# Themaister/Granite

Hardware: AMD Instinct MI355X
Metric: Mpixels/s for clustered-light+post chain @4K; achieved HBM GB/s vs roofline (higher is better)
Workload: dtype f32

## Files before the change

granite_amd/capi.py:

```python
from __future__ import annotations

import ctypes as C
import os
from typing import Optional

import numpy as np

_HERE = os.path.dirname(os.path.abspath(__file__))
LIB_PATH = os.path.join(_HERE, os.environ.get("GRANITE_LIB_DIR", "lib"), "libgranite_hip.so")

FORMAT_R8_UNORM = 9
FORMAT_R8G8_UNORM = 16
FORMAT_R8G8B8A8_UNORM = 37
FORMAT_R8G8B8A8_SRGB = 43
FORMAT_B8G8R8A8_UNORM = 44
FORMAT_B8G8R8A8_SRGB = 50
FORMAT_A2B10G10R10_UNORM_PACK32 = 64
FORMAT_R16_UNORM = 70
FORMAT_R16_SFLOAT = 76
FORMAT_R16G16_UNORM = 77
FORMAT_R16G16_SFLOAT = 83
FORMAT_R16G16B16A16_SFLOAT = 97
FORMAT_R32_SFLOAT = 100
FORMAT_R32G32_SFLOAT = 103
# ... 7 lines not shown
FORMAT_BC2_UNORM_BLOCK = 135
FORMAT_BC2_SRGB_BLOCK = 136
FORMAT_BC3_UNORM_BLOCK = 137
FORMAT_BC3_SRGB_BLOCK = 138
FORMAT_BC4_UNORM_BLOCK = 139
FORMAT_BC5_UNORM_BLOCK = 141
FORMAT_BC6H_UFLOAT_BLOCK = 143
FORMAT_BC6H_SFLOAT_BLOCK = 144
FORMAT_BC7_UNORM_BLOCK = 145
FORMAT_BC7_SRGB_BLOCK = 146
BLOCK_FORMATS = (131, 132, 133, 134, 135, 136, 137, 138, 139, 141, 143, 144, 145, 146)
FORMAT_ASTC_4x4_UNORM_BLOCK = 157
FORMAT_ASTC_4x4_SRGB_BLOCK = 158
FORMAT_ASTC_5x4_UNORM_BLOCK = 159
FORMAT_ASTC_5x4_SRGB_BLOCK = 160
FORMAT_ASTC_5x5_UNORM_BLOCK = 161
FORMAT_ASTC_5x5_SRGB_BLOCK = 162
FORMAT_ASTC_6x5_UNORM_BLOCK = 163
FORMAT_ASTC_6x5_SRGB_BLOCK = 164
FORMAT_ASTC_6x6_UNORM_BLOCK = 165
FORMAT_ASTC_6x6_SRGB_BLOCK = 166
FORMAT_ASTC_8x5_UNORM_BLOCK = 167
FORMAT_ASTC_8x5_SRGB_BLOCK = 168
FORMAT_ASTC_8x6_UNORM_BLOCK = 169
FORMAT_ASTC_8x6_SRGB_BLOCK = 170
FORMAT_ASTC_8x8_UNORM_BLOCK = 171
FORMAT_ASTC_8x8_SRGB_BLOCK = 172
FORMAT_ASTC_10x5_UNORM_BLOCK = 173
FORMAT_ASTC_10x5_SRGB_BLOCK = 174
FORMAT_ASTC_10x6_UNORM_BLOCK = 175
FORMAT_ASTC_10x6_SRGB_BLOCK = 176
FORMAT_ASTC_10x8_UNORM_BLOCK = 177
FORMAT_ASTC_10x8_SRGB_BLOCK = 178
FORMAT_ASTC_10x10_UNORM_BLOCK = 179
FORMAT_ASTC_10x10_SRGB_BLOCK = 180
FORMAT_ASTC_12x10_UNORM_BLOCK = 181
FORMAT_ASTC_12x10_SRGB_BLOCK = 182
FORMAT_ASTC_12x12_UNORM_BLOCK = 183
FORMAT_ASTC_12x12_SRGB_BLOCK = 184
ASTC_FOOTPRINTS = ((4, 4), (5, 4), (5, 5), (6, 5), (6, 6), (8, 5), (8, 6), (8, 8), (10, 5), (10, 6), (10, 8), (10, 10), (12, 10), (12, 12))
ASTC_FORMATS = {157 + i: ASTC_FOOTPRINTS[i // 2] for i in range(28)}

FORMAT_BPP = {
    FORMAT_R8_UNORM: 1,
    FORMAT_R8G8_UNORM: 2,
    FORMAT_R8G8B8A8_UNORM: 4,
    FORMAT_R8G8B8A8_SRGB: 4,
    FORMAT_B8G8R8A8_UNORM: 4,
    FORMAT_B8G8R8A8_SRGB: 4,
    FORMAT_R16_UNORM: 2,
    FORMAT_R16G16_UNORM: 4,
    FORMAT_A2B10G10R10_UNORM_PACK32: 4,
    FORMAT_R16_SFLOAT: 2,
    FORMAT_R16G16_SFLOAT: 4,
    FORMAT_R16G16B16A16_SFLOAT: 8,
    FORMAT_R32_SFLOAT: 4,
    FORMAT_R32G32_SFLOAT: 8,
    FORMAT_B10G11R11_UFLOAT_PACK32: 4,
    FORMAT_D16_UNORM: 2,
    FORMAT_D32_SFLOAT: 4,
}

COLOR_SPACE_SRGB_NONLINEAR = 0
COLOR_SPACE_EXTENDED_SRGB_LINEAR = 1000104002
COLOR_SPACE_HDR10_ST2084 = 1000104008
VIDEO_CONTROL_SKIP_RESCALE_BIT = 1
VIDEO_CONTROL_DOWNSCALING_BIT = 2
VIDEO_CONTROL_SAMPLED_DOWNSCALING_BIT = 4
VIDEO_CONTROL_CLAMP_COORD_BIT = 8
VIDEO_CONTROL_CHROMA_SUBSAMPLE_BIT = 16
VIDEO_CONTROL_PRIMARY_CONVERSION_BIT = 32
VIDEO_CONTROL_DITHER_BIT = 64
VIDEO_TRANSFER_IDENTITY = 0
VIDEO_TRANSFER_SRGB = 1
VIDEO_TRANSFER_PQ = 2
VIDEO_MATRIX_UNSPECIFIED, VIDEO_MATRIX_BT601_525, VIDEO_MATRIX_BT601_625, VIDEO_MATRIX_BT709, VIDEO_MATRIX_BT2020, VIDEO_MATRIX_SMPTE240M = range(6)
VIDEO_CHROMA_CENTER, VIDEO_CHROMA_LEFT, VIDEO_CHROMA_TOPLEFT, VIDEO_CHROMA_TOP, VIDEO_CHROMA_BOTTOMLEFT, VIDEO_CHROMA_BOTTOM = range(6)

LIGHTING_DIRECTIONAL_BIT = 1
LIGHTING_CLUSTERED_BIT = 2
LIGHTING_AMBIENT_FALLBACK_BIT = 4
LIGHTING_AMBIENT_OCCLUSION_BIT = 8
LIGHTING_SHARE_REGISTERS_BIT = 16

MAX_LIGHTS_BINDLESS = 4096
CULL_SETUP_BYTES_PER_LIGHT = 512
TRANSFORMED_SPOT_BYTES_PER_LIGHT = 96
TRANSFORMS_OFFSET_LIGHTS = 0
TRANSFORMS_OFFSET_SHADOW = 196608
TRANSFORMS_OFFSET_MODEL = 458752
TRANSFORMS_OFFSET_TYPE_MASK = 655360
TRANSFORMS_OFFSET_DECALS = 655872
TRANSFORMS_SIZE = 852480


class Cube(C.Structure):
    _fields_ = [("ptr", C.c_void_p), ("size", C.c_uint32), ("levels", C.c_uint32)]


class Image(C.Structure):
    _fields_ = [("ptr", C.c_void_p), ("width", C.c_uint32), ("height", C.c_uint32), ("pitch_bytes", C.c_uint32),
                ("format", C.c_uint32)]


FFT_FORWARD_C2C, FFT_INVERSE_C2C, FFT_R2C, FFT_C2R = 0, 1, 2, 3
FFT_FP32, FFT_FP16 = 0, 1
FFT_RESOURCE_TEXTURE, FFT_RESOURCE_BUFFER = 0, 1
FFT_PASS_C2C, FFT_PASS_R2C_RESOLVE, FFT_PASS_C2R_RESOLVE = 0, 1, 2
FFT_BUFFER_SRC, FFT_BUFFER_DST, FFT_BUFFER_SCRATCH_A, FFT_BUFFER_SCRATCH_B = 0, 1, 2, 3


class FftOptions(C.Structure):
    _fields_ = [("nx", C.c_uint32), ("ny", C.c_uint32), ("nz", C.c_uint32), ("dimensions", C.c_uint32), ("mode", C.c_uint32),
                ("data_type", C.c_uint32), ("input_resource", C.c_uint32), ("output_resource", C.c_uint32)]


class FftResource(C.Structure):
    _fields_ = [("type", C.c_uint32), ("ptr", C.c_void_p), ("size_bytes", C.c_uint64), ("row_stride", C.c_uint32), ("layer_stride", C.c_uint32),
                ("image", Image), ("output_offset", C.c_int32 * 2)]


class FftPass(C.Structure):
    _fields_ = [("kind", C.c_uint32), ("dimension", C.c_uint32), ("points", C.c_uint32), ("p", C.c_uint32), ("columns", C.c_uint32),
                ("workgroup_size", C.c_uint32), ("grid_size", C.c_uint32), ("lds_bytes", C.c_uint32), ("reads", C.c_uint32), ("writes", C.c_uint32)]


class PushVideo(C.Structure):
    _fields_ = [("resolution", C.c_int32 * 2), ("scaling_to_input", C.c_float * 2), ("inv_input_resolution", C.c_float * 2),
                ("dither_strength", C.c_float)]


assert C.sizeof(PushVideo) == 28


class VideoPlan(C.Structure):
    _fields_ = [("flags", C.c_uint32), ("eotf", C.c_uint32), ("oetf", C.c_uint32), ("num_planes", C.c_uint32), ("push", PushVideo),
                ("gamma_space_transform", C.c_float * 12), ("primary_transform", C.c_float * 9)]


class PushYuvToRgb(C.Structure):
    _fields_ = [("yuv_to_rgb", C.c_float * 16), ("primary_conversion", C.c_float * 16), ("resolution", C.c_uint32 * 2),
                ("inv_resolution", C.c_float * 2), ("chroma_siting", C.c_float * 2), ("chroma_clamp", C.c_float * 2),
                ("unorm_rescale", C.c_float)]


assert C.sizeof(PushYuvToRgb) == 164


class VideoYuvInfo(C.Structure):
    _fields_ = [("bit_depth", C.c_uint32), ("msb_aligned", C.c_uint32), ("full_range", C.c_uint32), ("matrix", C.c_uint32),
                ("chroma_location", C.c_uint32), ("pq", C.c_uint32), ("nv21", C.c_uint32)]


class VideoYuvPlan(C.Structure):
    _fields_ = [("push", PushYuvToRgb), ("spec_pq", C.c_uint32), ("spec_num_planes", C.c_uint32), ("spec_nv21", C.c_uint32),
                ("matrix", C.c_uint32)]


OCEAN_VARIANT_HEIGHT, OCEAN_VARIANT_GRADIENT_NORMAL, OCEAN_VARIANT_GRADIENT_DISPLACEMENT = 0, 1, 2
OCEAN_NUM_FREQ_BANDS = 8


class PushOceanGenerate(C.Structure):
    _fields_ = [("mod_factor", C.c_float * 2), ("N", C.c_uint32 * 2), ("freq_to_band_mod", C.c_float), ("time", C.c_float), ("period", C.c_float)]


# ... 1054 lines not shown
```

granite_amd/csrc/lighting.hip:

```cpp
#include <cstdlib>
#include <cstring>
#include "ctx.hpp"
#include "device_common.hpp"

namespace
{
constexpr int LIGHT_TILE = 8;
#ifndef LV_WAVES
#define LV_WAVES 4
#endif
constexpr int LIGHT_WAVES = LV_WAVES;
constexpr int LIGHT_SLOT_BYTES = 64;

constexpr float PI_SIC = 3.1415628f;
constexpr float CULL_RADIUS_SCALE = 1.001f;
constexpr float CULL_SLACK = 1e-3f;

#ifdef LV_STAMP
#define LV_STAMP_PARAM , uint32_t (&stamp_marks__)[4]
#define LV_STAMP_ARG , stamp_scope__.marks
#define LV_STAMP_MARK(k) stamp_marks__[k] = uint32_t(__builtin_amdgcn_s_memtime())
#define LV_STAMP_LAP_BEGIN() uint32_t stamp_lap__ = uint32_t(__builtin_amdgcn_s_memtime())
#define LV_STAMP_LAP(k)                                                          \
	do                                                                           \
// ... 75 lines not shown
__device__ __forceinline__ void brdf_accumulate(const Surface &s, float NdL, float hh, float scale, float3_ colour, float3_ &acc)
{
	const float NoL = med3(NdL, 0.001f, 1.0f);
	const float inv_h = rsq(hh);
	const float omh = sat(fmaf(-0.5f * hh, inv_h, 1.001f)) - 0.001f;
	const float NoH = sat((s.NdV + NdL) * inv_h);

	const float omh2 = omh * omh;
	const float f = omh2 * omh2 * omh;

	const float d = fmaf(NoH * NoH, s.m2m1, 1.0f);
	const float g = fmaf(NoL, s.gA, s.gB);
	const float GD = rcp(d * d * g);

	const float w = NoL * scale;
	const float cw = fmaf(-f, w, w);
	const float fw = f * GD * w;
	acc.x = fmaf(colour.x, fmaf(fmaf(GD, s.F0.x, s.D1.x), cw, fw), acc.x);
	acc.y = fmaf(colour.y, fmaf(fmaf(GD, s.F0.y, s.D1.y), cw, fw), acc.y);
	acc.z = fmaf(colour.z, fmaf(fmaf(GD, s.F0.z, s.D1.z), cw, fw), acc.z);
}

__device__ __forceinline__ bool index_in_range(uint32_t index, uint32_t range_x, uint32_t range_y)
{
	return index >= range_x && index <= range_y;
}

template <bool IS_MAX>
__device__ __forceinline__ uint32_t minmax_step(uint32_t v, uint32_t moved)
{
	return IS_MAX ? max(v, moved) : min(v, moved);
}
#define GR_DPP_STEP(IS_MAX, v, ctrl) v = minmax_step<IS_MAX>(v, uint32_t(__builtin_amdgcn_mov_dpp(int(v), ctrl, 0xf, 0xf, true)))
#define GR_DPP_BCAST(IS_MAX, v, ctrl, rows) \
	v = minmax_step<IS_MAX>(v, uint32_t(__builtin_amdgcn_update_dpp(IS_MAX ? 0 : -1, int(v), ctrl, rows, 0xf, false)))
template <bool IS_MAX>
__device__ __forceinline__ uint32_t wave_minmax_u32(uint32_t v)
{
	GR_DPP_STEP(IS_MAX, v, 0xB1);
	GR_DPP_STEP(IS_MAX, v, 0x4E);
	GR_DPP_STEP(IS_MAX, v, 0x141);
	GR_DPP_STEP(IS_MAX, v, 0x140);
	GR_DPP_BCAST(IS_MAX, v, 0x142, 0xa);
	GR_DPP_BCAST(IS_MAX, v, 0x143, 0xc);
	return uint32_t(__builtin_amdgcn_readlane(int(v), 63));
}
__device__ __forceinline__ void wave_min_and_max_u32(uint32_t &lo, uint32_t &hi)
{
	GR_DPP_STEP(false, lo, 0xB1);
	GR_DPP_STEP(true, hi, 0xB1);
	GR_DPP_STEP(false, lo, 0x4E);
	GR_DPP_STEP(true, hi, 0x4E);
	GR_DPP_STEP(false, lo, 0x141);
	GR_DPP_STEP(true, hi, 0x141);
	GR_DPP_STEP(false, lo, 0x140);
	GR_DPP_STEP(true, hi, 0x140);
	GR_DPP_BCAST(false, lo, 0x142, 0xa);
	GR_DPP_BCAST(true, hi, 0x142, 0xa);
	GR_DPP_BCAST(false, lo, 0x143, 0xc);
	GR_DPP_BCAST(true, hi, 0x143, 0xc);
	lo = uint32_t(__builtin_amdgcn_readlane(int(lo), 63));
	hi = uint32_t(__builtin_amdgcn_readlane(int(hi), 63));
}
#undef GR_DPP_STEP
#undef GR_DPP_BCAST

__device__ __forceinline__ uint32_t wave_inclusive_add_u32(uint32_t v)
{
	v += uint32_t(__builtin_amdgcn_update_dpp(0, int(v), 0x111, 0xf, 0xf, true));
	v += uint32_t(__builtin_amdgcn_update_dpp(0, int(v), 0x112, 0xf, 0xf, true));
	v += uint32_t(__builtin_amdgcn_update_dpp(0, int(v), 0x114, 0xf, 0xf, true));
	v += uint32_t(__builtin_amdgcn_update_dpp(0, int(v), 0x118, 0xf, 0xf, true));
	v += uint32_t(__builtin_amdgcn_update_dpp(0, int(v), 0x142, 0xa, 0xf, false));
	v += uint32_t(__builtin_amdgcn_update_dpp(0, int(v), 0x143, 0xc, 0xf, false));
	return v;
}
__device__ __forceinline__ uint32_t bits_from(uint32_t index, uint32_t word_first)
{
	return index <= word_first ? 0xffffffffu : (index - word_first >= 32u ? 0u : 0xffffffffu << (index - word_first));
}

extern __shared__ __attribute__((aligned(16))) uint8_t lv_dynamic_lds[];

template <int PX, bool CONE>
__device__ __forceinline__ void shade_positional(const Surface (&s)[PX], const f32x4 *slot, float3_ (&result)[PX])
{
	const f32x4 q0 = slot[0], q1 = slot[1];
	float3_ Lf[PX];
	float d2[PX];
	bool near_any = false;
#pragma unroll
	for (int p = 0; p < PX; p++)
	{
		Lf[p] = f3(q0.x, q0.y, q0.z) - s[p].pos;
		d2[p] = fmaf(Lf[p].z, Lf[p].z, fmaf(Lf[p].y, Lf[p].y, fmaf(Lf[p].x, Lf[p].x, 1e-30f)));
		near_any = near_any || d2[p] < q0.w;
	}
	if (!__any(near_any))
		return;

	float inv_d[PX], len[PX], inv_d2[PX], atten[PX];
#pragma unroll
	for (int p = 0; p < PX; p++)
	{
		inv_d[p] = rsq(d2[p]);
		len[p] = d2[p] * inv_d[p];
		const float dist = CONE ? fmaxf(0.1f, len[p]) : len[p];
		inv_d2[p] = inv_d[p] * inv_d[p];
		const float t = sat(fmaf(dist, q1.w, -9.0f));
		atten[p] = fmaf(t * t, fmaf(2.0f, t, -3.0f), 1.0f);
	}
	if (CONE)
	{
		const f32x4 q2 = slot[2], q3 = slot[3];
		bool lit_any = false;
#pragma unroll
		for (int p = 0; p < PX; p++)
		{
			const float cone_angle = -dot(Lf[p], f3(q2.x, q2.y, q2.z)) * inv_d[p];
			const float cone = sat(fmaf(cone_angle, q3.x, q3.y));
			atten[p] *= cone * cone;
			lit_any = lit_any || atten[p] > 0.0f;
		}
		if (!__any(lit_any))
			return;
	}
#pragma unroll
	for (int p = 0; p < PX; p++)
	{
		const float a2 = atten[p] * fminf(inv_d2[p], 1.0f / (0.1f * 0.1f));
		const float NdL = dot(s[p].N, Lf[p]) * inv_d[p];
		const float3_ Hs = f3(fmaf(s[p].V.x, len[p], Lf[p].x), fmaf(s[p].V.y, len[p], Lf[p].y), fmaf(s[p].V.z, len[p], Lf[p].z));
		const float hh = fmaf(Hs.z, Hs.z, fmaf(Hs.y, Hs.y, fmaf(Hs.x, Hs.x, 1e-30f))) * inv_d2[p];
		brdf_accumulate(s[p], NdL, hh, a2, f3(q1.x, q1.y, q1.z), result[p]);
	}
}


template <int PX, bool B10>
struct RawTile
{
	float depth[PX];
	uint32_t alb[PX], nrm[PX];
	uint32_t mr;
	uint32_t em[B10 ? PX : 2 * PX];
};

template <int PX, bool B10>
__device__ __forceinline__ void load_raw(const KernelArgs &a, int x0, int y, RawTile<PX, B10> &r)
{
	const uint32_t uy = uint32_t(min(y, a.hdr.h - 1)), ux = uint32_t(min(x0, a.hdr.w - PX));
	if constexpr (PX == 2)
	{
		const float2 d = *reinterpret_cast<const float2 *>(a.depth.ptr + (uy * a.depth.pitch + ux * 4u));
		const uint2 al = *reinterpret_cast<const uint2 *>(a.albedo.ptr + (uy * a.albedo.pitch + ux * 4u));
		const uint2 nr = *reinterpret_cast<const uint2 *>(a.normal.ptr + (uy * a.normal.pitch + ux * 4u));
		r.mr = *reinterpret_cast<const uint32_t *>(a.pbr.ptr + (uy * a.pbr.pitch + ux * 2u));
		if constexpr (B10)
		{
			const uint2 packed = *reinterpret_cast<const uint2 *>(a.emissive.ptr + (uy * a.emissive.pitch + ux * 4u));
			r.em[0] = packed.x, r.em[1] = packed.y;
		}
		else
		{
			const uint4 em = *reinterpret_cast<const uint4 *>(a.emissive.ptr + (uy * a.emissive.pitch + ux * 8u));
			r.em[0] = em.x, r.em[1] = em.y, r.em[2] = em.z, r.em[3] = em.w;
		}
		r.depth[0] = d.x, r.depth[PX - 1] = d.y;
		r.alb[0] = al.x, r.alb[PX - 1] = al.y;
		r.nrm[0] = nr.x, r.nrm[PX - 1] = nr.y;
	}
	else
	{
		r.depth[0] = *reinterpret_cast<const float *>(a.depth.ptr + (uy * a.depth.pitch + ux * 4u));
		r.alb[0] = *reinterpret_cast<const uint32_t *>(a.albedo.ptr + (uy * a.albedo.pitch + ux * 4u));
		r.nrm[0] = *reinterpret_cast<const uint32_t *>(a.normal.ptr + (uy * a.normal.pitch + ux * 4u));
		r.mr = *reinterpret_cast<const uint16_t *>(a.pbr.ptr + (uy * a.pbr.pitch + ux * 2u));
		if constexpr (B10)
			r.em[0] = *reinterpret_cast<const uint32_t *>(a.emissive.ptr + (uy * a.emissive.pitch + ux * 4u));
		else
		{
			const uint2 em = *reinterpret_cast<const uint2 *>(a.emissive.ptr + (uy * a.emissive.pitch + ux * 8u));
			r.em[0] = em.x, r.em[1] = em.y;
		}
	}
}


template <int PX, bool B10>
__device__ __forceinline__ void unpack_raw(const RawTile<PX, B10> &raw, float (&depth)[PX], uint32_t (&alb)[PX], uint32_t (&nrm)[PX], uint32_t (&mr)[PX],
                                           f16x4 (&dst)[PX])
{
#pragma unroll
	for (int p = 0; p < PX; p++)
	{
		depth[p] = raw.depth[p];
		alb[p] = raw.alb[p];
		nrm[p] = raw.nrm[p];
		mr[p] = PX == 2 ? (p == 0 ? raw.mr & 0xffffu : raw.mr >> 16) : raw.mr;
		if constexpr (B10)
		{
			uint32_t rg, ba;
			expand_b10g11r11(raw.em[p], rg, ba);
			dst[p] = __builtin_bit_cast(f16x4, make_uint2(rg, ba));
		}
		else
			dst[p] = __builtin_bit_cast(f16x4, make_uint2(raw.em[2 * p], raw.em[2 * p + 1]));
	}
}

template <bool B10, int CHANNEL>
__device__ __forceinline__ float blend_round(float v)
{
// ... 52 lines not shown
		const float3_ L = f3(a.dir_direction[0], a.dir_direction[1], a.dir_direction[2]);
		const float3_ Hv = s.V + L;
		float3_ lit = f3(0.0f, 0.0f, 0.0f);
		brdf_accumulate(s, dot(s.N, L), fmaxf(dot(Hv, Hv), 1e-30f), 1.0f, f3(a.dir_color[0], a.dir_color[1], a.dir_color[2]), lit);
		float ambient = (a.flags & GR_LIGHTING_AMBIENT_FALLBACK_BIT) ? 0.05f : 0.0f;
		if (AO)
			ambient *= sample_linear_r8(a.ao, (float(x) + 0.5f) * a.inv_resolution[0], (float(y) + 0.5f) * a.inv_resolution[1]);
		lit = f3(fmaf(base.x, ambient, lit.x), fmaf(base.y, ambient, lit.y), fmaf(base.z, ambient, lit.z));
		accum = f3(blend_round<B10, 0>(accum.x + lit.x), blend_round<B10, 1>(accum.y + lit.y), blend_round<B10, 2>(accum.z + lit.z));
	}
}

struct Cells { int cx0, cx1, cy0, cy1; };

__device__ __forceinline__ int cluster_cell(int p, float inv_res, float scale, int res)
{
	return clamp0_i32(int(__fmul_rn(__fmul_rn(float(p) + 0.5f, inv_res), scale)), res - 1);
}

template <int PX>
__device__ __forceinline__ Cells tile_cells(const KernelArgs &a, const int x0, const int y, const int lane)
{
	const int my_cx = cluster_cell(min(x0 + (lane >> 5) * (PX - 1), a.hdr.w - 1), a.inv_resolution[0], a.cl_xy_scale[0], a.cl_res_x);
	const int my_cy = cluster_cell(min(y, a.hdr.h - 1), a.inv_resolution[1], a.cl_xy_scale[1], a.cl_res_y);
	const int cx0 = __builtin_amdgcn_readlane(my_cx, 0), cx1 = __builtin_amdgcn_readlane(my_cx, 63);
	const int cy0 = __builtin_amdgcn_readlane(my_cy, 0), cy1 = __builtin_amdgcn_readlane(my_cy, 63);
	return {cx0, cx1, cy0, cy1};
}

template <int PX>
__device__ __forceinline__ void bounding_sphere(const bool (&member)[PX], const Surface (&s)[PX], float3_ &centre_out, float &radius_out)
{
	bool any_member = false;
#pragma unroll
	for (int p = 0; p < PX; p++)
		any_member = any_member || member[p];
	const int first = __builtin_ctzll(__ballot(any_member));
	const float3_ mine = PX == 2 && !member[0] ? s[PX - 1].pos : s[0].pos;
	centre_out = f3(__builtin_bit_cast(float, __builtin_amdgcn_readlane(__builtin_bit_cast(int, mine.x), first)),
	                __builtin_bit_cast(float, __builtin_amdgcn_readlane(__builtin_bit_cast(int, mine.y), first)),
	                __builtin_bit_cast(float, __builtin_amdgcn_readlane(__builtin_bit_cast(int, mine.z), first)));
	float off2 = 0.0f;
#pragma unroll
	for (int p = 0; p < PX; p++)
	{
		const float3_ off = s[p].pos - centre_out;
		const float mine2 = member[p] ? dot(off, off) : 0.0f;
		off2 = p == 0 ? mine2 : fmaxf(off2, mine2);
	}
	radius_out = __builtin_amdgcn_sqrtf(__builtin_bit_cast(float, wave_minmax_u32<true>(__builtin_bit_cast(uint32_t, off2)))) * 1.0001f + CULL_SLACK;
}

__device__ __forceinline__ void or_cell_words(const KernelArgs &a, const Cells &cells, const int my_word, uint32_t &word)
{
	for (int cy = cells.cy0; cy <= cells.cy1; cy++)
	{
#pragma clang loop vectorize(disable) unroll(disable)
		for (int cx = cells.cx0; cx <= cells.cx1; cx++)
			word |= a.bitmask[(cy * a.cl_res_x + cx) * a.cl_num_lights_32 + my_word];
	}
}

__device__ __forceinline__ int gather_wide(const KernelArgs &a, const Cells &cells, const uint32_t win_lo, const uint32_t win_hi, const uint32_t gap_lo,
                                           const uint32_t gap_hi, const int span_word, const int word_last, const int lane, uint16_t *const list)
{
	const int my_word = span_word + lane;
	const uint32_t word_first = uint32_t(my_word) << 5u;
	uint32_t word = 0u;
	if (lane < a.list_words && my_word <= word_last)
	{
		or_cell_words(a, cells, my_word, word);
		word &= bits_from(win_lo, word_first) & ~bits_from(win_hi + 1u, word_first) & ~(bits_from(gap_lo + 1u, word_first) & ~bits_from(gap_hi, word_first));
	}
	const uint32_t count = uint32_t(__builtin_popcount(word));
	const uint32_t upto = wave_inclusive_add_u32(count);
	const int list_count = __builtin_amdgcn_readlane(int(upto), 63);
	uint16_t *entry = list + (upto - count);
	for (; word != 0u; word &= word - 1u)
		*entry++ = uint16_t(word_first + uint32_t(__builtin_ctz(word)));
	__builtin_amdgcn_wave_barrier();
	return list_count;
}

__device__ __forceinline__ void cull_and_stage(const KernelArgs &a, const uint32_t light_index, const float3_ &centre, const float tile_radius, const int lane,
                                               f32x4 *const slots, bool &keep, bool &second)
{
	const f32x4 *rec = reinterpret_cast<const f32x4 *>(a.lights + light_index);
	const f32x4 c = rec[0], pq = rec[1], d = rec[2];
	const float radius = CULL_RADIUS_SCALE * rcp(d.w);
	const float3_ to_light = f3(pq.x, pq.y, pq.z) - centre;
	const float reach = radius + tile_radius;
	const float dist2 = dot(to_light, to_light);
	keep = dist2 <= reach * reach;
	const bool is_spot = ((a.type_mask[light_index >> 5] >> (light_index & 31u)) & 1u) == 0u;
	const float sb_lane = c.w;
	const uint32_t sb_bits = __builtin_bit_cast(uint32_t, sb_lane);
	const float spot_scale = float(__builtin_bit_cast(_Float16, uint16_t(sb_bits & 0xffffu)));
	const float spot_bias = float(__builtin_bit_cast(_Float16, uint16_t(sb_bits >> 16)));
	if (is_spot && keep && spot_scale > 0.0f)
	{
		const float cos_t = -spot_bias * rcp(spot_scale);
		if (cos_t > 0.0f && cos_t < 1.0f)
		{
			const float sin_t = __builtin_amdgcn_sqrtf(fmaf(-cos_t, cos_t, 1.0f));
			const float along = -dot(to_light, f3(d.x, d.y, d.z));
			const float off_axis = __builtin_amdgcn_sqrtf(fmaxf(fmaf(-along, along, dist2), 0.0f));
			const float e = fmaf(off_axis, cos_t, -along * sin_t);
			keep = e <= tile_radius * 1.001f + CULL_SLACK;
		}
	}
	second = is_spot || d.w > 8.0f;
	if (keep)
	{
		f32x4 *dst_slot = slots + lane * (LIGHT_SLOT_BYTES / 16);
		dst_slot[0] = f32x4{pq.x, pq.y, pq.z, radius * radius};
		dst_slot[1] = f32x4{c.x, c.y, c.z, 10.0f * d.w};
		if (second)
		{
			dst_slot[2] = is_spot ? f32x4{d.x, d.y, d.z, 0.0f} : f32x4{0.0f, 0.0f, 0.0f, 0.0f};
			dst_slot[3] = is_spot ? f32x4{spot_scale, spot_bias, 0.0f, 0.0f} : f32x4{0.0f, 1.0f, 0.0f, 0.0f};
		}
	}
}

template <int PX, bool CONE>
__device__ __forceinline__ void walk_next(uint64_t &todo, const Surface (&s)[PX], const f32x4 *const slots, float3_ (&result)[PX])
{
	const int bit = __builtin_ctzll(todo);
	asm("s_bitset0_b64 %0, %1" : "+s"(todo) : "s"(bit));
	shade_positional<PX, CONE>(s, slots + bit * (LIGHT_SLOT_BYTES / 16), result);
}

template <int PX, bool AO, bool B10>
__device__ __forceinline__ void shade_tile(const KernelArgs &a, const int tile_x0, const int tile_y0, const int wave, const int lane, const RawTile<PX, B10> &raw,
                                           f32x4 *const slots, const float *s_srgb LV_STAMP_PARAM)
{
	const int x0 = tile_x0 + (lane & (LIGHT_TILE - 1)) * PX;
	const int y = tile_y0 + (lane >> 3);
	const int W = a.hdr.w;
	const bool row_inside = y >= a.row_first && y < a.row_end;

	bool inside[PX], active[PX];
#pragma unroll
	for (int p = 0; p < PX; p++)
		inside[p] = row_inside && x0 + p < W;
	f16x4 dst[PX];
	float depth[PX];
	uint32_t alb[PX], nrm[PX], mr[PX];
	unpack_raw<PX, B10>(raw, depth, alb, nrm, mr, dst);
	float clip_base[4];
	{
		const float ndc_x = fmaf(2.0f * (float(x0) + 0.5f), a.inv_resolution[0], -1.0f);
		const float ndc_y = fmaf(2.0f * (float(y) + 0.5f), a.inv_resolution[1], -1.0f);
#pragma unroll
		for (int i = 0; i < 4; i++)
			clip_base[i] = fmaf(a.inv_vp[4 + i], ndc_y, fmaf(a.inv_vp[i], ndc_x, a.inv_vp[12 + i]));
	}

	Surface s[PX];
	float3_ accum[PX];
	bool any_active = false;
#pragma unroll
	for (int p = 0; p < PX; p++)
	{
		active[p] = inside[p] && depth[p] != 0.0f;
		any_active = any_active || active[p];
		float3_ base, N;
		float metallic, mat_roughness;
		decode_gbuffer(alb[p], nrm[p], mr[p], s_srgb, base, N, metallic, mat_roughness);
		float clip[4];
#pragma unroll
		for (int i = 0; i < 4; i++)
			clip[i] = fmaf(depth[p], a.inv_vp[8 + i], p == 0 ? clip_base[i] : clip_base[i] + float(p) * a.clip_dx[i]);
		make_surface(a, clip, active[p], N, base, metallic, mat_roughness, s[p]);
		accum[p] = f3(float(dst[p].x), float(dst[p].y), float(dst[p].z));
		directional_quad<AO, B10>(a, s[p], base, x0 + p, y, accum[p]);
	}

	LV_STAMP_MARK(0);
	f16x4 out_h[PX];
	float3_ out_f[PX];
	if ((a.flags & GR_LIGHTING_CLUSTERED_BIT) && a.cl_num_lights > 0)
	{
		float3_ result[PX];
		uint32_t lane_lo = 0xffffffffu, lane_hi = 0u;
		uint2 px_range[PX];
#pragma unroll
		for (int p = 0; p < PX; p++)
		{
			result[p] = f3(0.0f, 0.0f, 0.0f);
			const float zf = fmaf(s[p].pos.z, a.cl_z_row[2], fmaf(s[p].pos.y, a.cl_z_row[1], fmaf(s[p].pos.x, a.cl_z_row[0], a.cl_z_row[3])));
			const uint32_t z_index = uint32_t(clamp0_i32(int(zf), a.cl_z_max_index));
			if (active[p])
			{
				const uint2 z_range = *reinterpret_cast<const uint2 *>(reinterpret_cast<const uint8_t *>(a.range) + (z_index << 3u));
				px_range[p] = z_range;
				lane_lo = min(lane_lo, z_range.x);
				lane_hi = max(lane_hi, z_range.y);
			}
		}
		wave_min_and_max_u32(lane_lo, lane_hi);
		const uint32_t win_lo = lane_lo, win_hi = min(lane_hi, uint32_t(a.cl_num_lights - 1));
		const bool wide = a.list_words != 0 && win_lo <= win_hi && (win_hi >> 6u) - (win_lo >> 6u) >= 2u;
		uint32_t gap_lo = 0u, gap_hi = 0xffffffffu;
		bool in_low[PX], in_high[PX];
#pragma unroll
		for (int p = 0; p < PX; p++)
			in_low[p] = in_high[p] = false;
		if (wide)
		{
			uint32_t first_end = 0xffffffffu;
#pragma unroll
			for (int p = 0; p < PX; p++)
				first_end = min(first_end, active[p] && px_range[p].x <= px_range[p].y ? px_range[p].y : 0xffffffffu);
			first_end = wave_minmax_u32<false>(first_end);
#pragma unroll
			for (int p = 0; p < PX; p++)
			{
				const bool some = active[p] && px_range[p].x <= px_range[p].y, low = px_range[p].x <= first_end;
				in_low[p] = some && low, in_high[p] = some && !low;
				gap_lo = max(gap_lo, some && low ? px_range[p].y : 0u);
				gap_hi = min(gap_hi, some && !low ? px_range[p].x : 0xffffffffu);
			}
			wave_min_and_max_u32(gap_hi, gap_lo);
		}
		if (win_lo <= win_hi)
		{
			const Cells cells = tile_cells<PX>(a, x0, y, lane);
			float3_ centre;
			float tile_radius;
			bounding_sphere<PX>(active, s, centre, tile_radius);

			LV_STAMP_MARK(1);
			LV_STAMP_LAP_BEGIN();
			const int chunk_lo = int(win_lo >> 6u), chunk_hi = int(win_hi >> 6u);
			auto turn = [&](const uint32_t light_index, const bool candidate, const float3_ &centre, const float tile_radius) __attribute__((always_inline)) {
				bool keep = false, second = false;
				if (candidate)
					cull_and_stage(a, light_index, centre, tile_radius, lane, slots, keep, second);
				const uint64_t kept = __ballot(keep);
				const uint64_t seconds = __ballot(keep && second);
				__builtin_amdgcn_wave_barrier();
				LV_STAMP_LAP(2);

				for (uint64_t todo = kept & ~seconds; todo != 0ull;)
					walk_next<PX, false>(todo, s, slots, result);
				for (uint64_t todo = seconds; todo != 0ull;)
					walk_next<PX, true>(todo, s, slots, result);
				LV_STAMP_LAP(3);
				__builtin_amdgcn_wave_barrier();
			};
			if (!wide)
			{
				for (int chunk = chunk_lo; chunk <= chunk_hi; chunk++)
				{
					const uint32_t light_index = uint32_t(chunk) * 64u + uint32_t(lane);
					const int my_word = chunk * 2 + (lane >> 5);
					bool candidate = false;
					if (index_in_range(light_index, win_lo, win_hi))
					{
						uint32_t word = 0u;
						or_cell_words(a, cells, my_word, word);
						candidate = ((word >> (uint32_t(lane) & 31u)) & 1u) != 0u;
					}
					turn(light_index, candidate, centre, tile_radius);
				}
			}
			else
			{
				const bool two_groups = gap_hi != 0xffffffffu && gap_hi > gap_lo + 1u;
				float3_ centre_low = centre, centre_high = centre;
				float radius_low = tile_radius, radius_high = tile_radius;
				if (two_groups)
				{
					bounding_sphere<PX>(in_low, s, centre_low, radius_low);
					bounding_sphere<PX>(in_high, s, centre_high, radius_high);
				}
				uint16_t *const list = reinterpret_cast<uint16_t *>(lv_dynamic_lds) + wave * (a.list_words * 32);
				const int word_last = int(win_hi >> 5u);
				for (int span_word = int(win_lo >> 5u); span_word <= word_last; span_word += a.list_words)
				{
					const int list_count = gather_wide(a, cells, win_lo, win_hi, gap_lo, gap_hi, span_word, word_last, lane, list);
					for (int next = 0; next < list_count; next += 64)
					{
						const bool candidate = next + lane < list_count;
						const uint32_t light_index = candidate ? uint32_t(list[next + lane]) : 0u;
						const bool upper = light_index >= gap_hi;
						turn(light_index, candidate,
						     f3(upper ? centre_high.x : centre_low.x, upper ? centre_high.y : centre_low.y, upper ? centre_high.z : centre_low.z),
						     upper ? radius_high : radius_low);
					}
					__builtin_amdgcn_wave_barrier();
				}
			}
		}
#pragma unroll
		for (int p = 0; p < PX; p++)
		{
			out_f[p] = f3(accum[p].x + result[p].x, accum[p].y + result[p].y, accum[p].z + result[p].z);
			out_h[p].x = _Float16(out_f[p].x);
			out_h[p].y = _Float16(out_f[p].y);
			out_h[p].z = _Float16(out_f[p].z);
		}
	}
	else
	{
#pragma unroll
		for (int p = 0; p < PX; p++)
		{
			out_f[p] = accum[p];
			out_h[p].x = _Float16(accum[p].x);
			out_h[p].y = _Float16(accum[p].y);
			out_h[p].z = _Float16(accum[p].z);
		}
	}

	if (!inside[0])
		return;
	f16x4 o[PX];
#pragma unroll
	for (int p = 0; p < PX; p++)
	{
		o[p] = dst[p];
		if (active[p])
		{
			o[p].x = out_h[p].x;
			o[p].y = out_h[p].y;
			o[p].z = out_h[p].z;
		}
	}
	if (a.fog_falloff > 0.0f)
	{
#pragma unroll
		for (int p = 0; p < PX; p++)
			if (active[p])
			{
				const float3_ eye = s[p].pos - f3(a.camera_pos[0], a.camera_pos[1], a.camera_pos[2]);
				const float f = __builtin_amdgcn_exp2f(-dot(eye, eye) * a.fog_falloff), omf = 1.0f - f;
				const float3_ lit = B10 ? f3(round_to_ufloat<6>(out_f[p].x), round_to_ufloat<6>(out_f[p].y), round_to_ufloat<5>(out_f[p].z))
				                        : f3(float(o[p].x), float(o[p].y), float(o[p].z));
				out_f[p] = f3(fmaf(lit.x, f, a.fog_color[0] * omf), fmaf(lit.y, f, a.fog_color[1] * omf), fmaf(lit.z, f, a.fog_color[2] * omf));
				o[p].x = _Float16(out_f[p].x);
				o[p].y = _Float16(out_f[p].y);
				o[p].z = _Float16(out_f[p].z);
				o[p].w = _Float16(fmaf(float(dst[p].w), f, f * omf));
			}
	}
	if constexpr (B10)
	{
		if (any_active || a.emissive.ptr != a.hdr.ptr)
		{
			uint32_t words[PX];
#pragma unroll
			for (int p = 0; p < PX; p++)
				words[p] = active[p] ? pack_b10g11r11(out_f[p].x, out_f[p].y, out_f[p].z) : pack_b10g11r11(float(dst[p].x), float(dst[p].y), float(dst[p].z));
			uint8_t *out = a.hdr.ptr + (uint32_t(y) * a.hdr.pitch + uint32_t(x0) * 4u);
			if constexpr (PX == 2)
				*reinterpret_cast<uint2 *>(out) = make_uint2(words[0], words[PX - 1]);
			else
				*reinterpret_cast<uint32_t *>(out) = words[0];
		}
		return;
	}
	if (any_active || a.emissive.ptr != a.hdr.ptr)
	{
		uint8_t *out = a.hdr.ptr + (uint32_t(y) * a.hdr.pitch + uint32_t(x0) * 8u);
		if constexpr (PX == 2)
		{
			const uint2 lo = __builtin_bit_cast(uint2, o[0]), hi = __builtin_bit_cast(uint2, o[PX - 1]);
			*reinterpret_cast<uint4 *>(out) = make_uint4(lo.x, lo.y, hi.x, hi.y);
		}
		else
			*reinterpret_cast<f16x4 *>(out) = o[0];
// ... 22 lines not shown
		asm volatile("s_getreg_b32 %0, hwreg(HW_REG_HW_ID)" : "=s"(hw));
		if (rec && (threadIdx.x & 63u) == 0u)
		{
			rec[0] = make_uint4(uint32_t(t0), uint32_t(t1), uint32_t(c1 - c0), (xcc << 28) | (hw & 0x0fffffffu));
			rec[1] = make_uint4(marks[0] ? marks[0] - uint32_t(c0) : 0u, marks[1] ? marks[1] - uint32_t(c0) : 0u, marks[2], marks[3]);
		}
	}
};
#define LV_STAMP_SCOPE(tile) StampScope stamp_scope__{uint32_t(tile)}
#else
#define LV_STAMP_SCOPE(tile)
#endif

#ifdef LV_WAVES_PER_EU
#define LV_OCCUPANCY_ATTR __attribute__((amdgpu_waves_per_eu(LV_WAVES_PER_EU, LV_WAVES_PER_EU)))
#else
#define LV_OCCUPANCY_ATTR
#endif
template <int PX, bool AO, bool B10 = false>
__global__ __launch_bounds__(64 * LIGHT_WAVES) LV_OCCUPANCY_ATTR void k_lighting(KernelArgs a)
{
	__shared__ __attribute__((aligned(16))) f32x4 s_lights[LIGHT_WAVES][64 * (LIGHT_SLOT_BYTES / 16)];
	__shared__ float s_srgb[256];
	constexpr int TILE_W = LIGHT_TILE * PX;
#pragma unroll
	for (int i = 0; i < 256; i += 64 * LIGHT_WAVES)
		s_srgb[i + threadIdx.x] = a.srgb_lut[i + threadIdx.x];
	const int wave = __builtin_amdgcn_readfirstlane(int(threadIdx.x >> 6));
	const int lane = threadIdx.x & 63;
	const int tile_x0 = (int(blockIdx.x) * LIGHT_WAVES + wave) * TILE_W, tile_y0 = (a.block_row0 + int(blockIdx.y)) * LIGHT_TILE;
	LV_STAMP_SCOPE((int(blockIdx.y) * int(gridDim.x) + int(blockIdx.x)) * LIGHT_WAVES + wave);
	RawTile<PX, B10> raw;
	load_raw<PX, B10>(a, tile_x0 + (lane & (LIGHT_TILE - 1)) * PX, tile_y0 + (lane >> 3), raw);
	__syncthreads();
	shade_tile<PX, AO, B10>(a, tile_x0, tile_y0, wave, lane, raw, s_lights[threadIdx.x >> 6], s_srgb LV_STAMP_ARG);
}

KernelArgs fill_kernel_args(const gr_lighting_args *args, const gr_ctx *ctx, const bool clustered)
{
	KernelArgs k{};
	k.albedo = to_dev(&args->albedo);
	k.normal = to_dev(&args->normal);
	k.pbr = to_dev(&args->pbr);
	k.depth = to_dev(&args->depth);
	k.emissive = to_dev(&args->emissive);
	if (args->flags & GR_LIGHTING_AMBIENT_OCCLUSION_BIT)
		k.ao = to_dev(&args->ambient_occlusion);
	k.hdr = to_dev_rw(&args->hdr);
	for (int i = 0; i < 16; i++)
		k.inv_vp[i] = args->inv_view_projection[i];
	for (int i = 0; i < 4; i++)
		k.clip_dx[i] = k.inv_vp[i] * (2.0f * args->clustering.inv_resolution[0]);
	for (int i = 0; i < 3; i++)
	{
		k.camera_pos[i] = args->clustering.camera_pos[i];
		k.dir_color[i] = args->directional.color[i];
		k.dir_direction[i] = args->directional.direction[i];
	}
	k.inv_resolution[0] = args->clustering.inv_resolution[0];
	k.inv_resolution[1] = args->clustering.inv_resolution[1];
	k.cl_xy_scale[0] = args->cluster.xy_scale[0];
	k.cl_xy_scale[1] = args->cluster.xy_scale[1];
	k.cl_res_x = args->cluster.resolution_xy[0];
	k.cl_res_y = args->cluster.resolution_xy[1];
	k.cl_num_lights = clustered ? args->cluster.num_lights : 0;
	k.cl_num_lights_32 = args->cluster.num_lights_32;
	k.cl_z_max_index = args->cluster.z_max_index;
	{
		const float *front = args->cluster.camera_front, *camera = args->cluster.camera_base;
		const double z_scale = args->cluster.z_scale;
		for (int i = 0; i < 3; i++)
			k.cl_z_row[i] = float(double(front[i]) * z_scale);
		k.cl_z_row[3] = float(-(double(camera[0]) * front[0] + double(camera[1]) * front[1] + double(camera[2]) * front[2]) * z_scale);
	}
	if (clustered)
	{
		const uint8_t *t = static_cast<const uint8_t *>(args->transforms);
		k.lights = reinterpret_cast<const gr_light_info *>(t + GR_TRANSFORMS_OFFSET_LIGHTS);
		k.type_mask = reinterpret_cast<const uint32_t *>(t + GR_TRANSFORMS_OFFSET_TYPE_MASK);
		k.bitmask = args->bitmask;
		k.range = reinterpret_cast<const uint2 *>(args->range);
	}
	k.srgb_lut = ctx->srgb_decode_lut;
	k.flags = args->flags & (GR_LIGHTING_DIRECTIONAL_BIT | GR_LIGHTING_CLUSTERED_BIT | GR_LIGHTING_AMBIENT_FALLBACK_BIT | GR_LIGHTING_AMBIENT_OCCLUSION_BIT);
	for (int i = 0; i < 3; i++)
		k.fog_color[i] = args->fog_color[i];
	k.fog_falloff = args->fog_falloff > 0.0f ? args->fog_falloff : 0.0f;
	return k;
}

struct LdsPolicy
{
	size_t pad_lds;
	int list_words;
};
LdsPolicy lds_policy(const int px, const uint32_t flags)
{
	static const int max_wgs_env = []() {
		const char *env = gr_measurement_switch("GR_LIGHTING_WGS_PER_CU");
		const int v = env ? atoi(env) : 0;
		return v >= 1 && v <= 8 ? v : 0;
	}();
	const int max_wgs = max_wgs_env ? max_wgs_env : (px == 2 ? ((flags & GR_LIGHTING_SHARE_REGISTERS_BIT) ? 4 : 5) : 7);
	const size_t static_lds = sizeof(f32x4) * LIGHT_WAVES * 64 * (LIGHT_SLOT_BYTES / 16) + 256 * sizeof(float);
	const size_t per_wg = ((160u - 8u) * 1024u / unsigned(max_wgs * 4 / LIGHT_WAVES)) & ~size_t(1023);
	LdsPolicy lds{max_wgs >= 8 || per_wg <= static_lds ? 0 : per_wg - static_lds, 0};
	static const int pad_kib = []() { const char *env = gr_measurement_switch("GR_LIGHTING_PAD_KIB"); return env ? atoi(env) : -1; }();
	if (pad_kib >= 0)
		lds.pad_lds = size_t(pad_kib) * 1024u;
	const size_t words = lds.pad_lds / (size_t(LIGHT_WAVES) * 32u * sizeof(uint16_t));
	static const bool narrow_only = []() { const char *env = gr_measurement_switch("GR_LIGHTING_NARROW_ONLY"); return env && atoi(env) != 0; }();
	if (words >= 8 && !narrow_only)
		lds.list_words = int(words < 64 ? words : 64);
	return lds;
}

}

extern "C" {

int gr_lighting(gr_ctx *ctx, gr_stream stream, const gr_lighting_args *args)
{
	if (!ctx)
		return GR_ERR_INVALID_ARGUMENT;
	GR_CHECK_ARG(ctx, args != nullptr);
	GR_CHECK_IMAGE(ctx, &args->hdr, GR_HDR_FORMATS);
	const uint32_t W = args->hdr.width, H = args->hdr.height;
	const bool b10 = args->hdr.format == GR_FORMAT_B10G11R11_UFLOAT_PACK32;
	const uint32_t hdr_bpp = gr_format_texel_bytes(args->hdr.format);
	GR_CHECK_IMAGE(ctx, &args->emissive, args->hdr.format, W, H);
	GR_CHECK_IMAGE(ctx, &args->albedo, GR_FORMAT_R8G8B8A8_SRGB, W, H);
	GR_CHECK_IMAGE(ctx, &args->normal, GR_FORMAT_A2B10G10R10_UNORM_PACK32, W, H);
	GR_CHECK_IMAGE(ctx, &args->pbr, GR_FORMAT_R8G8_UNORM, W, H);
	GR_CHECK_IMAGE(ctx, &args->depth, GR_FORMAT_D32_SFLOAT, W, H);
	const bool clustered = (args->flags & GR_LIGHTING_CLUSTERED_BIT) != 0 && args->cluster.num_lights > 0;
	if (clustered)
	{
		GR_CHECK_ARG(ctx, args->transforms && args->bitmask && args->range);
		GR_CHECK_ARG(ctx, args->cluster.num_lights <= GR_MAX_LIGHTS_BINDLESS);
		GR_CHECK_ARG(ctx, args->cluster.resolution_xy[0] > 0 && args->cluster.resolution_xy[1] > 0);
	}

	const bool ao = (args->flags & GR_LIGHTING_AMBIENT_OCCLUSION_BIT) != 0;
	if (ao)
	{
		GR_CHECK_ARG(ctx, (args->flags & GR_LIGHTING_AMBIENT_FALLBACK_BIT) != 0);
		GR_CHECK_IMAGE(ctx, &args->ambient_occlusion, GR_FORMAT_R8_UNORM);
	}
	const RowSpan span = resolve_rows(args->rows.count ? &args->rows : nullptr, H);
	if (span.count() == 0)
		return GR_OK;
	GR_CHECK_ARG(ctx, uint64_t(args->hdr.pitch_bytes) * H <= 0xffffffffull && uint64_t(args->emissive.pitch_bytes) * H <= 0xffffffffull);

	KernelArgs k = fill_kernel_args(args, ctx, clustered);
	k.row_first = int(span.first);
	k.row_end = int(span.end);
	k.block_row0 = int(span.first / LIGHT_TILE);
	static const int px_pref = []() {
		const char *env = gr_measurement_switch("GR_LIGHTING_PX");
		return env && atoi(env) == 1 ? 1 : 2;
	}();
	const bool pairs_aligned = (W & 1u) == 0 && is_aligned(&args->depth, 8u) && is_aligned(&args->albedo, 8u) && is_aligned(&args->normal, 8u) &&
	                           is_aligned(&args->pbr, 4u) && is_aligned(&args->emissive, 2u * hdr_bpp) && is_aligned(&args->hdr, 2u * hdr_bpp);
	const int px = pairs_aligned ? px_pref : 1;
	const LdsPolicy lds = lds_policy(px, args->flags);
	k.list_words = lds.list_words;

// ... 22 lines not shown
```

include/granite_hip.h:

```cpp
#ifndef GRANITE_HIP_H_
#define GRANITE_HIP_H_

#include <stddef.h>
#include <stdint.h>

#ifdef __cplusplus
extern "C" {
#endif

#define GR_ABI_VERSION 1

typedef struct gr_ctx gr_ctx;
typedef void *gr_stream;

typedef enum gr_status
{
	GR_OK = 0,
	GR_ERR_INVALID_ARGUMENT = -1,
	GR_ERR_HIP = -2,
	GR_ERR_UNSUPPORTED_FORMAT = -3,
	GR_ERR_OUT_OF_MEMORY = -4
} gr_status;

typedef enum gr_format
// ... 267 lines not shown
#define GR_TRANSFORMS_OFFSET_TYPE_MASK 655360u
#define GR_TRANSFORMS_OFFSET_DECALS 655872u
#define GR_TRANSFORMS_SIZE 852480u

typedef struct gr_push_spot_transform
{
	float vp[16];
	float camera_pos[3];
	uint32_t num_lights;
	float camera_front[3];
	float z_near;
	float z_far;
} gr_push_spot_transform;
int gr_cluster_spot_transform(gr_ctx *ctx, gr_stream stream, const void *transforms, void *transformed_spots,
                              const gr_push_spot_transform *push);

typedef struct gr_push_cluster_setup
{
	float view[16];
	uint32_t num_lights;
} gr_push_cluster_setup;
int gr_cluster_setup(gr_ctx *ctx, gr_stream stream, const void *transforms, const void *transformed_spots,
                     void *cull_setup, const gr_cluster_params *params, const gr_push_cluster_setup *push);

int gr_cluster_binning(gr_ctx *ctx, gr_stream stream, const void *transforms, const void *cull_setup, uint32_t *bitmask,
                       const gr_cluster_params *params);

typedef struct gr_push_z_range
{
	uint32_t num_volumes;
	uint32_t num_volumes_128;
	uint32_t num_ranges;
} gr_push_z_range;
int gr_cluster_z_range(gr_ctx *ctx, gr_stream stream, const uint32_t *light_ranges, uint32_t *out,
                       const gr_push_z_range *push);

typedef struct gr_cluster_front_args
{
	void *transforms;
	const void *src_lights;
	const void *src_models;
	const void *src_type_mask;
	void *transformed_spots;
	void *cull_setup;
	const gr_cluster_params *params;
	const gr_push_spot_transform *spot_push;
	const gr_push_cluster_setup *setup_push;
	const void *src_ranges;
	uint32_t *light_ranges;
	uint32_t *range_out;
	const gr_push_z_range *z_push;
} gr_cluster_front_args;
int gr_cluster_front(gr_ctx *ctx, gr_stream stream, const gr_cluster_front_args *args);

typedef struct gr_push_directional
{
	float inv_view_proj_col2[4];
	float color[3];
	float environment_intensity;
	float camera_pos[3];
	float environment_mipscale;
	float direction[3];
	float cascade_log_bias;
	float camera_front[3];
	float pad0;
	float inv_resolution[2];
	float pad1[2];
} gr_push_directional;

typedef struct gr_push_clustering
{
	float inv_view_proj_col2[4];
	float camera_pos[3];
	float pad0;
	float inv_resolution[2];
	float pad1[2];
} gr_push_clustering;

#define GR_LIGHTING_DIRECTIONAL_BIT 1u
#define GR_LIGHTING_CLUSTERED_BIT 2u
#define GR_LIGHTING_AMBIENT_FALLBACK_BIT 4u
#define GR_LIGHTING_AMBIENT_OCCLUSION_BIT 8u
#define GR_LIGHTING_SHARE_REGISTERS_BIT 16u

typedef struct gr_lighting_args
{
	gr_image albedo;
	gr_image normal;
	gr_image pbr;
	gr_image depth;
	gr_image emissive;
	gr_image hdr;
	float inv_view_projection[16];
	gr_push_directional directional;
	gr_push_clustering clustering;
	gr_cluster_params cluster;
	const void *transforms;
	const uint32_t *bitmask;
	const uint32_t *range;
	uint32_t flags;
	gr_rows rows;
	gr_image ambient_occlusion;
	float fog_color[3];
	float fog_falloff;
} gr_lighting_args;
int gr_lighting(gr_ctx *ctx, gr_stream stream, const gr_lighting_args *args);

int gr_pack_rgb8_rows(gr_ctx *ctx, gr_stream stream, const gr_image *image, const gr_rows *rows, void *packed);
int gr_unpack_rgb8_rows(gr_ctx *ctx, gr_stream stream, const void *packed, const gr_image *image, const gr_rows *rows);

int gr_blit(gr_ctx *ctx, gr_stream stream, const gr_image *in, const gr_image *out, int linear);


typedef struct gr_push_fxaa
{
	float inv_resolution[2];
} gr_push_fxaa;
int gr_fxaa(gr_ctx *ctx, gr_stream stream, const gr_image *in, const gr_image *out, const gr_push_fxaa *push);
int gr_fxaa_rows(gr_ctx *ctx, gr_stream stream, const gr_image *in, const gr_image *out, const gr_push_fxaa *push, const gr_rows *rows);

typedef struct gr_push_smaa
{
	float rt_metrics[4];
} gr_push_smaa;
int gr_smaa_set_luts(gr_ctx *ctx, const void *area_rg8, const void *search_r8);
int gr_smaa_edge_detection(gr_ctx *ctx, gr_stream stream, const gr_image *color, const gr_image *edges, const gr_push_smaa *push, int quality);
int gr_smaa_blend_weight(gr_ctx *ctx, gr_stream stream, const gr_image *edges, const gr_image *weights, const gr_push_smaa *push, int quality);
int gr_smaa_neighbor_blend(gr_ctx *ctx, gr_stream stream, const gr_image *color, const gr_image *weights, const gr_image *out,
                           const gr_push_smaa *push);
int gr_smaa_edge_detection_rows(gr_ctx *ctx, gr_stream stream, const gr_image *color, const gr_image *edges, const gr_push_smaa *push,
                                int quality, const gr_rows *rows);
int gr_smaa_blend_weight_rows(gr_ctx *ctx, gr_stream stream, const gr_image *edges, const gr_image *weights, const gr_push_smaa *push,
                              int quality, const gr_rows *rows);
int gr_smaa_neighbor_blend_rows(gr_ctx *ctx, gr_stream stream, const gr_image *color, const gr_image *weights, const gr_image *out,
                                const gr_push_smaa *push, const gr_rows *rows);
typedef struct gr_push_taa
{
	float reproj[16];
	float rt_metrics[4];
} gr_push_taa;
int gr_taa_resolve(gr_ctx *ctx, gr_stream stream, const gr_image *current, const gr_image *depth, const gr_image *mv,
                   const gr_image *history, const gr_image *out_color, const gr_image *out_history, const gr_push_taa *push, int quality);
int gr_taa_resolve_rows(gr_ctx *ctx, gr_stream stream, const gr_image *current, const gr_image *depth, const gr_image *mv,
                        const gr_image *history, const gr_image *out_color, const gr_image *out_history, const gr_push_taa *push, int quality,
                        const gr_rows *rows);
int gr_taa_resolve_band(gr_ctx *ctx, gr_stream stream, const gr_image *current, const gr_image *depth, const gr_image *mv,
                        const gr_image *history, const gr_image *out_color, const gr_image *out_history, const gr_push_taa *push, int quality,
                        const gr_rows *rows, const gr_rows *history_rows, uint32_t *reach_flag);

size_t gr_mip_chain_offset(uint32_t width, uint32_t height, uint32_t bytes_per_texel, uint32_t level);
size_t gr_mip_chain_size(uint32_t width, uint32_t height, uint32_t bytes_per_texel, uint32_t levels);

typedef struct gr_hiz_args
{
	gr_image depth;
	void *chain;
	uint32_t chain_width;
	uint32_t chain_height;
	uint32_t chain_levels;
	uint32_t output_downsample;
	float z_transform[4];
	uint32_t *counter;
} gr_hiz_args;
int gr_hiz(gr_ctx *ctx, gr_stream stream, const gr_hiz_args *args);

typedef struct gr_ssr_args
// ... 780 lines not shown
```

Before: 41370.

## Add interior fast path for point lights fully covering a tile

During culling, each point light is classified as 'interior' when the whole tile sits well inside its radius but outside the near clamp distance. Such lights are shaded with a specialised path that drops the range early-out, the smoothstep attenuation and the min clamp. The walk over kept point lights alternates runs of interior and general lights using scalar find-first-bit. This adds a classification cost per light and more code paths, which could raise register pressure. A new flag can disable the interior classification.

```diff
diff --git a/granite_amd/capi.py b/granite_amd/capi.py
--- a/granite_amd/capi.py
+++ b/granite_amd/capi.py
@@ -113,6 +113,7 @@
 LIGHTING_AMBIENT_FALLBACK_BIT = 4
 LIGHTING_AMBIENT_OCCLUSION_BIT = 8
 LIGHTING_SHARE_REGISTERS_BIT = 16
+LIGHTING_GENERAL_WALK_BIT = 32
 
 MAX_LIGHTS_BINDLESS = 4096
 CULL_SETUP_BYTES_PER_LIGHT = 512
diff --git a/granite_amd/csrc/lighting.hip b/granite_amd/csrc/lighting.hip
--- a/granite_amd/csrc/lighting.hip
+++ b/granite_amd/csrc/lighting.hip
@@ -181,9 +181,10 @@
 
 extern __shared__ __attribute__((aligned(16))) uint8_t lv_dynamic_lds[];
 
-template <int PX, bool CONE>
+template <int PX, bool CONE, bool INTERIOR = false>
 __device__ __forceinline__ void shade_positional(const Surface (&s)[PX], const f32x4 *slot, float3_ (&result)[PX])
 {
+	static_assert(!(CONE && INTERIOR), "the cone walk has no interior form");
 	const f32x4 q0 = slot[0], q1 = slot[1];
 	float3_ Lf[PX];
 	float d2[PX];
@@ -193,10 +194,14 @@
 	{
 		Lf[p] = f3(q0.x, q0.y, q0.z) - s[p].pos;
 		d2[p] = fmaf(Lf[p].z, Lf[p].z, fmaf(Lf[p].y, Lf[p].y, fmaf(Lf[p].x, Lf[p].x, 1e-30f)));
-		near_any = near_any || d2[p] < q0.w;
-	}
-	if (!__any(near_any))
-		return;
+		if constexpr (!INTERIOR)
+			near_any = near_any || d2[p] < q0.w;
+	}
+	if constexpr (!INTERIOR)
+	{
+		if (!__any(near_any))
+			return;
+	}
 
 	float inv_d[PX], len[PX], inv_d2[PX], atten[PX];
 #pragma unroll
@@ -204,10 +209,19 @@
 	{
 		inv_d[p] = rsq(d2[p]);
 		len[p] = d2[p] * inv_d[p];
-		const float dist = CONE ? fmaxf(0.1f, len[p]) : len[p];
 		inv_d2[p] = inv_d[p] * inv_d[p];
-		const float t = sat(fmaf(dist, q1.w, -9.0f));
-		atten[p] = fmaf(t * t, fmaf(2.0f, t, -3.0f), 1.0f);
+		if constexpr (!INTERIOR)
+		{
+			const float dist = CONE ? fmaxf(0.1f, len[p]) : len[p];
+			const float t = sat(fmaf(dist, q1.w, -9.0f));
+			atten[p] = fmaf(t * t, fmaf(2.0f, t, -3.0f), 1.0f);
+		}
+	}
+	if constexpr (INTERIOR && PX == 2)
+	{
+		typedef float f32x2 __attribute__((ext_vector_type(2)));
+		const f32x2 both = f32x2{d2[0], d2[PX - 1]} * f32x2{inv_d[0], inv_d[PX - 1]};
+		len[0] = both.x, len[PX - 1] = both.y;
 	}
 	if (CONE)
 	{
@@ -227,7 +241,7 @@
 #pragma unroll
 	for (int p = 0; p < PX; p++)
 	{
-		const float a2 = atten[p] * fminf(inv_d2[p], 1.0f / (0.1f * 0.1f));
+		const float a2 = INTERIOR ? inv_d2[p] : atten[p] * fminf(inv_d2[p], 1.0f / (0.1f * 0.1f));
 		const float NdL = dot(s[p].N, Lf[p]) * inv_d[p];
 		const float3_ Hs = f3(fmaf(s[p].V.x, len[p], Lf[p].x), fmaf(s[p].V.y, len[p], Lf[p].y), fmaf(s[p].V.z, len[p], Lf[p].z));
 		const float hh = fmaf(Hs.z, Hs.z, fmaf(Hs.y, Hs.y, fmaf(Hs.x, Hs.x, 1e-30f))) * inv_d2[p];
@@ -446,16 +460,19 @@
 	return list_count;
 }
 
-__device__ __forceinline__ void cull_and_stage(const KernelArgs &a, const uint32_t light_index, const float3_ &centre, const float tile_radius, const int lane,
-                                               f32x4 *const slots, bool &keep, bool &second)
+__device__ __forceinline__ void cull_and_stage(const KernelArgs &a, const uint32_t light_index, const float3_ &centre, const float tile_radius,
+                                               const bool whole_tile, const int lane, f32x4 *const slots, bool &keep, bool &second, bool &interior)
 {
 	const f32x4 *rec = reinterpret_cast<const f32x4 *>(a.lights + light_index);
 	const f32x4 c = rec[0], pq = rec[1], d = rec[2];
-	const float radius = CULL_RADIUS_SCALE * rcp(d.w);
+	const float true_radius = rcp(d.w);
+	const float radius = CULL_RADIUS_SCALE * true_radius;
 	const float3_ to_light = f3(pq.x, pq.y, pq.z) - centre;
 	const float reach = radius + tile_radius;
 	const float dist2 = dot(to_light, to_light);
 	keep = dist2 <= reach * reach;
+	const float within = fmaf(true_radius, 0.8999f, -tile_radius), beyond = tile_radius + 0.11f;
+	interior = whole_tile && within >= 0.0f && dist2 <= within * within && dist2 >= beyond * beyond;
 	const bool is_spot = ((a.type_mask[light_index >> 5] >> (light_index & 31u)) & 1u) == 0u;
 	const float sb_lane = c.w;
 	const uint32_t sb_bits = __builtin_bit_cast(uint32_t, sb_lane);
@@ -474,6 +491,7 @@
 		}
 	}
 	second = is_spot || d.w > 8.0f;
+	interior = interior && !second;
 	if (keep)
 	{
 		f32x4 *dst_slot = slots + lane * (LIGHT_SLOT_BYTES / 16);
@@ -487,12 +505,43 @@
 	}
 }
 
-template <int PX, bool CONE>
+template <int PX, bool CONE, bool INTERIOR = false>
 __device__ __forceinline__ void walk_next(uint64_t &todo, const Surface (&s)[PX], const f32x4 *const slots, float3_ (&result)[PX])
 {
 	const int bit = __builtin_ctzll(todo);
 	asm("s_bitset0_b64 %0, %1" : "+s"(todo) : "s"(bit));
-	shade_positional<PX, CONE>(s, slots + bit * (LIGHT_SLOT_BYTES / 16), result);
+	shade_positional<PX, CONE, INTERIOR>(s, slots + bit * (LIGHT_SLOT_BYTES / 16), result);
+}
+__device__ __forceinline__ uint32_t lowest_bit_or_none(uint64_t mask)
+{
+	uint32_t bit;
+	asm("s_ff1_i32_b64 %0, %1" : "=s"(bit) : "s"(mask));
+	return bit;
+}
+
+template <int PX>
+__device__ __forceinline__ void walk_points(const uint64_t points, const uint64_t interiors, const Surface (&s)[PX], const f32x4 *const slots,
+                                            float3_ (&result)[PX])
+{
+	uint64_t todo = points;
+	uint32_t bit = lowest_bit_or_none(todo);
+	while (todo != 0ull)
+	{
+		uint32_t stop = lowest_bit_or_none(todo & ~interiors);
+		while (bit < stop)
+		{
+			asm("s_bitset0_b64 %0, %1" : "+s"(todo) : "s"(bit));
+			shade_positional<PX, false, true>(s, slots + bit * (LIGHT_SLOT_BYTES / 16), result);
+			bit = lowest_bit_or_none(todo);
+		}
+		stop = lowest_bit_or_none(todo & interiors);
+		while (bit < stop)
+		{
+			asm("s_bitset0_b64 %0, %1" : "+s"(todo) : "s"(bit));
+			shade_positional<PX, false>(s, slots + bit * (LIGHT_SLOT_BYTES / 16), result);
+			bit = lowest_bit_or_none(todo);
+		}
+	}
 }
 
 template <int PX, bool AO, bool B10>
@@ -598,17 +647,17 @@
 			LV_STAMP_MARK(1);
 			LV_STAMP_LAP_BEGIN();
 			const int chunk_lo = int(win_lo >> 6u), chunk_hi = int(win_hi >> 6u);
-			auto turn = [&](const uint32_t light_index, const bool candidate, const float3_ &centre, const float tile_radius) __attribute__((always_inline)) {
-				bool keep = false, second = false;
+			auto turn = [&](const uint32_t light_index, const bool candidate, const float3_ &centre, const float tile_radius, const bool whole_tile) __attribute__((always_inline)) {
+				bool keep = false, second = false, interior = false;
 				if (candidate)
-					cull_and_stage(a, light_index, centre, tile_radius, lane, slots, keep, second);
+					cull_and_stage(a, light_index, centre, tile_radius, whole_tile, lane, slots, keep, second, interior);
 				const uint64_t kept = __ballot(keep);
 				const uint64_t seconds = __ballot(keep && second);
+				const uint64_t interiors = (a.flags & GR_LIGHTING_GENERAL_WALK_BIT) ? 0ull : __ballot(keep && interior);
 				__builtin_amdgcn_wave_barrier();
 				LV_STAMP_LAP(2);
 
-				for (uint64_t todo = kept & ~seconds; todo != 0ull;)
-					walk_next<PX, false>(todo, s, slots, result);
+				walk_points<PX>(kept & ~seconds, interiors, s, slots, result);
 				for (uint64_t todo = seconds; todo != 0ull;)
 					walk_next<PX, true>(todo, s, slots, result);
 				LV_STAMP_LAP(3);
@@ -627,7 +676,7 @@
 						or_cell_words(a, cells, my_word, word);
 						candidate = ((word >> (uint32_t(lane) & 31u)) & 1u) != 0u;
 					}
-					turn(light_index, candidate, centre, tile_radius);
+					turn(light_index, candidate, centre, tile_radius, true);
 				}
 			}
 			else
@@ -652,7 +701,7 @@
 						const bool upper = light_index >= gap_hi;
 						turn(light_index, candidate,
 						     f3(upper ? centre_high.x : centre_low.x, upper ? centre_high.y : centre_low.y, upper ? centre_high.z : centre_low.z),
-						     upper ? radius_high : radius_low);
+						     upper ? radius_high : radius_low, !two_groups);
 					}
 					__builtin_amdgcn_wave_barrier();
 				}
@@ -841,7 +890,8 @@
 		k.range = reinterpret_cast<const uint2 *>(args->range);
 	}
 	k.srgb_lut = ctx->srgb_decode_lut;
-	k.flags = args->flags & (GR_LIGHTING_DIRECTIONAL_BIT | GR_LIGHTING_CLUSTERED_BIT | GR_LIGHTING_AMBIENT_FALLBACK_BIT | GR_LIGHTING_AMBIENT_OCCLUSION_BIT);
+	k.flags = args->flags & (GR_LIGHTING_DIRECTIONAL_BIT | GR_LIGHTING_CLUSTERED_BIT | GR_LIGHTING_AMBIENT_FALLBACK_BIT | GR_LIGHTING_AMBIENT_OCCLUSION_BIT |
+	                         GR_LIGHTING_GENERAL_WALK_BIT);
 	for (int i = 0; i < 3; i++)
 		k.fog_color[i] = args->fog_color[i];
 	k.fog_falloff = args->fog_falloff > 0.0f ? args->fog_falloff : 0.0f;
diff --git a/include/granite_hip.h b/include/granite_hip.h
--- a/include/granite_hip.h
+++ b/include/granite_hip.h
@@ -373,6 +373,7 @@
 #define GR_LIGHTING_AMBIENT_FALLBACK_BIT 4u
 #define GR_LIGHTING_AMBIENT_OCCLUSION_BIT 8u
 #define GR_LIGHTING_SHARE_REGISTERS_BIT 16u
+#define GR_LIGHTING_GENERAL_WALK_BIT 32u
 
 typedef struct gr_lighting_args
 {
```

New measurement: 42090 (median of 4 runs). 1.7% higher.
